# jnez71/lqRRT

Hardware: AMD Instinct MI355X
Metric: tree-node extensions/sec, 6-DoF boat, 10k-node tree (higher is better)
Workload: dtype f64; 1 GPU; demo_boat_advanced_10k; wave_cap=256, wave_cap_cli=1024, semantics=exact-sequential, parallelism=single GPU

## Files before the change

### lqrrt_amd/csrc/steer.hpp

```cpp
#pragma once

template <class S, class = void> struct is_packed : std::false_type {};
template <class S> struct is_packed<S, std::enable_if_t<S::PACKED>> : std::true_type {};

__device__ __forceinline__ bool uniform_true(bool b) { return __builtin_amdgcn_readfirstlane((int)b) != 0; }

struct SteerFuse {
    const Part* part; int n_chunks;
    NodeView nv; const double* Sd; long long s_stride;
    unsigned char* changed; unsigned char* stale; int* par_out;
    double* M; int W;
    const double* xtrig;
    int* lf0; int* round_ctl;
    double* sh_hdr; double* sh_tail; int* sh_cursor; int sh_hd, sh_tb;
};

template <class S, class = void> struct wants_two : std::false_type {};
template <class S> struct wants_two<S, std::enable_if_t<S::TWO_WAVEFRONTS>> : std::true_type {};
template <class S> constexpr int steer_wavefronts_max() { return has_dare_gain<S>::value ? 4 : is_packed<S>::value ? 3 : wants_two<S>::value ? 2 : 1; }
struct DuoLds {
    double pk[2 * MAXN + 4 + MAXM];
    double rud;
    int go, stop, cnt, steps, grew, truncated;
    int fin;
    double pk2[2][2 * MAXN + 4 + MAXM];
    double tr[2][2];
    double e2b[2];
    double tt[2];
};

template <class S>
__device__ __forceinline__ void rollout_record(const double* xn, const double* trn, const double* u, int cnt,
                                               double* hx, double* hu, double* htr) {
#pragma unroll
    for (int d = 0; d < S::N; ++d) hx[cnt * S::N + d] = xn[d];
#pragma unroll
    for (int j = 0; j < S::M; ++j) hu[cnt * S::M + j] = u[j];
#pragma unroll
    for (int j = 0; j < 2 * S::NW; ++j) htr[2 * S::NW * cnt + j] = trn[j];
}
template <class S>
__device__ __forceinline__ bool rollout_check(const double* Pl, const Geo& g, const GeoL& gl, const Res& r, const double* xn,
                                              const double* trn, const double* e, const double* u, int lane, int& cnt, int& steps,
                                              double* last, const double* tolr, double* hx, double* hu, double* htr, DuoLds& duo,
                                              bool* rec_later = nullptr, const bool* feas_known = nullptr) {
    bool stop = false;
    const bool feas_ok = feas_known ? *feas_known : uniform_true(S::feasible(Pl, g, gl, xn, u, trn, lane));
    if (!feas_ok) {
        cnt = (int)(r.FPR * (double)cnt);
        duo.truncated = 1;
        stop = true;
    } else {
        ++steps;
        if (r.adaptive) {
            bool all_grew = true;
#pragma unroll
            for (int d = 0; d < S::N; ++d) all_grew = all_grew && (fabs(e[d]) >= last[d]);
            if (uniform_true(all_grew)) { cnt = 0; duo.grew = 1; stop = true; }
#pragma unroll
            for (int d = 0; d < S::N; ++d) last[d] = fabs(e[d]);
        }
        if (!stop) {
            bool conv = true;
#pragma unroll
            for (int d = 0; d < S::N; ++d) conv = conv && (fabs(e[d]) <= tolr[d]);
            if (steps > r.H || uniform_true(conv)) {
                stop = true;
            } else {
                if (rec_later) *rec_later = true;
                else { rollout_record<S>(xn, trn, u, cnt, hx, hu, htr); ++cnt; }
            }
        }
    }
    if (stop) { duo.cnt = cnt; duo.steps = steps; duo.stop = 1; }
    return stop;
}

template <class S, int DENSE, int NWF, bool KERNARG_TOUCH>
__device__ __forceinline__ void steer_body(const Params& P, const Geo& g, const Res& r, const TreeView& tv, double* __restrict__ rec,
                                           const RecLayout& L, const double* __restrict__ xs,
                                           const int* __restrict__ list, const int lo,
                                           const int* __restrict__ par, const int* __restrict__ list_count,
                                           const SteerFuse& f, const RoundArgs& ra, const int rd_on, const int rd_round, const int rd_W, const int rd_base, const int rd_seq, const long long rd_max_commit, const long long rd_room, const int bid) {
    const bool ron = rd_on != 0;
    if (list_count && bid + lo >= list_count[0]) return;
#ifndef LQRRT_NO_KERNARG_TOUCH
    if constexpr (KERNARG_TOUCH) {
        const volatile int* ka = (const volatile int*)__builtin_amdgcn_kernarg_segment_ptr();
        constexpr int KA_LINES = (int)((sizeof(Params) + sizeof(Geo) + sizeof(Res) + sizeof(TreeView) + sizeof(RecLayout) +
                                        sizeof(SteerFuse) + sizeof(RoundArgs) + 40) / 64);
        if ((int)(threadIdx.x & 63) < KA_LINES) (void)ka[(threadIdx.x & 63) * 16];
    }
#endif
    STEER_TS(0);
    BLK_T(blk_t0);
    constexpr bool COOP = has_dare_gain<S>::value && NWF == 4;
    constexpr int GNT = COOP ? 256 : 64;
    constexpr bool DUO = NWF >= 2 && !COOP;
    static_assert(NWF <= 2 || is_packed<S>::value || COOP, "the chain rollout needs the duo_* / *_effort pieces of the system");
    static_assert(!has_dare_gain<S>::value || NWF == 1 || NWF == 4, "Riccati systems: one wavefront, or four that share the gain");
    constexpr bool PLAIN2 = NWF == 2 && !is_packed<S>::value;
    extern __shared__ double hist[];
    double* hx = hist;
    double* hu = hist + (size_t)r.H * S::N;
    const int lane = threadIdx.x & 63;
    __shared__ double Pl[MAXP];
    __shared__ double tol_l[MAXN], glo_l[MAXN], ghi_l[MAXN];
    __shared__ double node_l[MAXN + 4 + MAXM * MAXN];
    __shared__ GainLds<S> gl_lds;
    __shared__ DuoLds duo;
    double* htr = hist + (size_t)r.H * (S::N + S::M) + geo_lds_doubles(g);
    constexpr int PKN = S::N + 2 * S::NW;
    constexpr bool CH = NWF == 3 && is_packed<S>::value;
    if constexpr (CH) {
        if (threadIdx.x >= 128) {
            if (ron && !ra.gblk && ra.ctl[RC_CONV + (rd_round & 1)]) return;
            for (int i = lane; i < MAXP; i += 64) Pl[i] = P.p[i];
            if (lane < MAXN) { tol_l[lane] = r.tol[lane]; glo_l[lane] = r.goal_lo[lane]; ghi_l[lane] = r.goal_hi[lane]; }
            const GeoL gl = stage_geo(g, hist + (size_t)r.H * (S::N + S::M), lane, 64);
            __syncthreads();
            if (!duo.go) return;
            double tolr[S::N], last[S::N];
#pragma unroll
            for (int d = 0; d < S::N; ++d) { tolr[d] = tol_l[d]; last[d] = INFINITY; }
            int cnt = 0, steps = 0;
            bool stopped = false;
            for (int p = 1;; ++p) {
                __syncthreads();
                if (stopped) return;
                STEP_TS(cs0);
                double xn[S::N], trn[2], e[S::N], u[S::M];
                const double* pk = duo.pk2[p & 1];
#pragma unroll
                for (int d = 0; d < S::N; ++d) { xn[d] = pk[d]; e[d] = pk[S::N + d]; }
#pragma unroll
                for (int j = 0; j < S::M; ++j) u[j] = pk[2 * S::N + j];
                trn[0] = duo.tr[p & 1][0]; trn[1] = duo.tr[p & 1][1];
                bool rec_now = false;
                stopped = rollout_check<S>(Pl, g, gl, r, xn, trn, e, u, lane, cnt, steps, last, tolr, hx, hu, htr, duo, &rec_now);
                if (rec_now) { rollout_record<S>(xn, trn, u, cnt, hx, hu, htr); ++cnt; }
                STEP_TS(cs1);
                STEP_ACC(5, cs0, cs1);
            }
        }
        if (threadIdx.x >= 64) {
            if (ron && !ra.gblk && ra.ctl[RC_CONV + (rd_round & 1)]) return;
            __syncthreads();
            if (!duo.go) return;
            const double tt0 = duo.tt[0], tt1 = duo.tt[1];
            for (int p = 0;; ++p) {
                STEP_TS(ds0);
                const double hn = duo.pk2[p & 1][2] + duo.pk2[p & 1][5] * r.dt;
                double tn[2];
                lq_sincos(hn, &tn[1], &tn[0]);
                duo.tr[(p + 1) & 1][0] = tn[0]; duo.tr[(p + 1) & 1][1] = tn[1];
                duo.e2b[(p + 1) & 1] = lq_atan2(tt1 * tn[0] - tt0 * tn[1], tt0 * tn[0] + tt1 * tn[1]);
                STEP_TS(ds1);
                STEP_ACC(7, ds0, ds1);
                __syncthreads();
                if (duo.stop) return;
            }
        }
    }
    if constexpr (PLAIN2) {
        if (threadIdx.x >= 64) {
            if (ron && !ra.gblk && ra.ctl[RC_CONV + (rd_round & 1)]) return;
            for (int i = lane; i < MAXP; i += 64) Pl[i] = P.p[i];
            if (lane < MAXN) { tol_l[lane] = r.tol[lane]; glo_l[lane] = r.goal_lo[lane]; ghi_l[lane] = r.goal_hi[lane]; }
            const GeoL gl = stage_geo(g, hist + (size_t)r.H * (S::N + S::M), lane, 64);
            __syncthreads();
            if (!duo.go) return;
            double tolr[S::N], last[S::N];
#pragma unroll
            for (int d = 0; d < S::N; ++d) { tolr[d] = tol_l[d]; last[d] = INFINITY; }
            int cnt = 0, steps = 0;
            for (int k = 0;; ++k) {
                __syncthreads();
                if (duo.stop) return;
                double xn[S::N], trn[2 * S::NW + 1], e[S::N], u[S::M];
                const double* pk = duo.pk2[k & 1];
#pragma unroll
                for (int d = 0; d < S::N; ++d) { xn[d] = pk[d]; e[d] = pk[PKN + d]; }
#pragma unroll
                for (int j = 0; j < 2 * S::NW; ++j) trn[j] = pk[S::N + j];
#pragma unroll
                for (int j = 0; j < S::M; ++j) u[j] = pk[PKN + S::N + j];
                rollout_check<S>(Pl, g, gl, r, xn, trn, e, u, lane, cnt, steps, last, tolr, hx, hu, htr, duo);
            }
        }
    }
    if constexpr (NWF == 2 && !PLAIN2) {
        if (threadIdx.x >= 64) {
            if (ron && !ra.gblk && ra.ctl[RC_CONV + (rd_round & 1)]) return;
            for (int i = lane; i < MAXP; i += 64) Pl[i] = P.p[i];
            if (lane < MAXN) { tol_l[lane] = r.tol[lane]; glo_l[lane] = r.goal_lo[lane]; ghi_l[lane] = r.goal_hi[lane]; }
            const GeoL gl = stage_geo(g, hist + (size_t)r.H * (S::N + S::M), lane, 64);
            __syncthreads();
            if (!duo.go) return;
            double tolr[S::N], last[S::N];
#pragma unroll
            for (int d = 0; d < S::N; ++d) { tolr[d] = tol_l[d]; last[d] = INFINITY; }
            int cnt = 0, steps = 0;
            for (int k = 0;; ++k) {
                double xn[S::N], trn[2], e[S::N], u[S::M];
                STEP_TS(hs0);
#pragma unroll
                for (int d = 0; d < S::N; ++d) { xn[d] = duo.pk[d]; e[d] = duo.pk[S::N + 2 + d]; }
                trn[0] = duo.pk[S::N]; trn[1] = duo.pk[S::N + 1];
#pragma unroll
                for (int j = 0; j < S::M; ++j) u[j] = duo.pk[2 * S::N + 2 + j];
                if (!duo.fin) duo.rud = S::duo_chain(Pl, xn, trn);
                STEP_TS(hs1);
                __syncthreads();
                STEP_TS(hs2);
                if (k >= 1) {
                    bool stop = false;
                    const bool feas_ok = uniform_true(S::feasible(Pl, g, gl, xn, u, trn, lane));
                    if (!feas_ok) {
                        cnt = (int)(r.FPR * (double)cnt);
                        duo.truncated = 1;
                        stop = true;
                    } else {
                        ++steps;
                        if (r.adaptive) {
                            bool all_grew = true;
#pragma unroll
                            for (int d = 0; d < S::N; ++d) all_grew = all_grew && (fabs(e[d]) >= last[d]);
                            if (uniform_true(all_grew)) { cnt = 0; duo.grew = 1; stop = true; }
#pragma unroll
                            for (int d = 0; d < S::N; ++d) last[d] = fabs(e[d]);
                        }
                        if (!stop) {
                            bool conv = true;
#pragma unroll
                            for (int d = 0; d < S::N; ++d) conv = conv && (fabs(e[d]) <= tolr[d]);
                            if (steps > r.H || uniform_true(conv)) {
                                stop = true;
                            } else {
#pragma unroll
                                for (int d = 0; d < S::N; ++d) hx[cnt * S::N + d] = xn[d];
#pragma unroll
                                for (int j = 0; j < S::M; ++j) hu[cnt * S::M + j] = u[j];
                                htr[2 * cnt] = trn[0]; htr[2 * cnt + 1] = trn[1];
                                ++cnt;
                            }
                        }
                    }
                    if (stop) { duo.cnt = cnt; duo.steps = steps; duo.stop = 1; }
                }
                STEP_TS(hs3);
                __syncthreads();
                STEP_TS(hs4);
                STEP_ACC(0, hs0, hs1); STEP_ACC(1, hs1, hs2); STEP_ACC(2, hs2, hs3); STEP_ACC(4, hs3, hs4); STEP_ACC(3, hs0, hs0 + 1);
                if (duo.stop) return;
            }
        }
    }
    const int t = list ? list[bid + (list_count ? lo : 0)] : lo + bid;
    double* my = rec + (size_t)t * L.R;

    double x[S::N], K[S::M * S::N], trig[2 * S::NW + 1], xt[S::N], ttrig[2 * S::NW + 1];
#pragma unroll
    for (int d = 0; d < S::N; ++d) xt[d] = xs[(size_t)t * S::N + d];
    if (f.xtrig) {
#pragma unroll
        for (int j = 0; j < 2 * S::NW; ++j) ttrig[j] = f.xtrig[(size_t)t * (2 * S::NW) + j];
    } else {
        trig_of<S>(xt, ttrig);
    }
    bool parent_loaded = false;
    constexpr int HD = S::N + 2 * S::NW + S::M * S::N;
    int psel = 0;
    int head_out = 0;
    auto load_parent = [&](int p) {
        if (p >= 0) {
#pragma unroll
            for (int d = 0; d < S::N; ++d) x[d] = tv.state[(size_t)d * tv.cap + p];
#pragma unroll
            for (int j = 0; j < 2 * S::NW; ++j) trig[j] = tv.trig[(size_t)j * tv.cap + p];
#pragma unroll
            for (int j = 0; j < S::M * S::N; ++j) K[j] = tv.K[(size_t)p * S::M * S::N + j];
        } else {
            const double* hp = (ron && ra.gblk) ? gathered_header(ra, ~p) + L.off_xend
                             : (ron && psel)    ? ra.head2 + (size_t)(~p) * HD
                                                : rec + (size_t)(~p) * L.R + L.off_xend;
#pragma unroll
            for (int d = 0; d < S::N; ++d) x[d] = hp[d];
#pragma unroll
            for (int j = 0; j < 2 * S::NW; ++j) trig[j] = hp[S::N + j];
#pragma unroll
            for (int j = 0; j < S::M * S::N; ++j) K[j] = hp[S::N + 2 * S::NW + j];
        }
// ... 116 lines not shown
            stale_t = ra.stale[cur][t];
        }
        auto flags_of = [&](int idx) -> int {
            int v = 0;
#pragma unroll
            for (int i = 0; i < 4; ++i) { const int w = __shfl((int)chg[i], idx & 63); if ((idx >> 6) == i) v = w; }
            return v;
        };
        auto changed_of = [&](int idx) -> bool { return (flags_of(idx) & 1) != 0; };
        auto sel_of = [&](int idx) -> int { return (flags_of(idx) >> 1) & 1; };
        const int sel_t = sel_of(t);
        if (conv_flag) {
            const int C = ra.ctl[RC_C];
            const int len = ra.lf[cur][2 * t];
            if (t < C && len > 0) {
                const int id = rd_base + ra.rank[t];
                const double* hd = sel_t ? ra.head2 + (size_t)t * HD : my + L.off_xend;
                if (lane < S::N) tv.state[(size_t)lane * tv.cap + id] = hd[lane];
                if (lane < 2 * S::NW) tv.trig[(size_t)lane * tv.cap + id] = hd[S::N + lane];
                if constexpr (S::NW > 0) {
                    if (ra.fx.on && lane >= 32 && lane < 32 + S::NW) {
                        const int kk = lane - 32;
                        tv.werr[(size_t)kk * tv.cap + id] = wrap_err(ra.fx.t[2 * kk], ra.fx.t[2 * kk + 1], hd[S::N + 2 * kk], hd[S::N + 2 * kk + 1]);
                    }
                }
                for (int q = lane; q < S::M * S::N; q += 64) tv.K[(size_t)id * S::M * S::N + q] = hd[S::N + 2 * S::NW + q];
                if (lane == 0) {
                    const int p = ra.par[cur][t];
                    tv.pID[id] = p >= 0 ? p : rd_base + ra.rank[~p];
                    tv.elen[id] = len;
                }
                double* xe = tv.xedge + (size_t)id * tv.H * S::N;
                double* ue = tv.uedge + (size_t)id * tv.H * S::M;
                for (int q = lane; q < len * S::N; q += 64) xe[q] = my[L.off_xseq + q];
                for (int q = lane; q < len * S::M; q += 64) ue[q] = my[L.off_useq + q];
            }
            return;
        }
        int want = par_t;
        bool need = false, defer = false, mark_stale = false;
        int hz = rd_W - 1;
#pragma unroll
        for (int i = 0; i < 4; ++i)
            if (hz == rd_W - 1 && lf_len[i] > 0 && (lf_flg[i] & 1)) hz = lane + 64 * i;
#pragma unroll
        for (int off = 32; off > 0; off >>= 1) hz = min(hz, __shfl_xor(hz, off));
        if (t <= hz) {
            double wc = INFINITY;
            int sm = -1;
#pragma unroll
            for (int i = 0; i < 4; ++i)
                if (lane + 64 * i < t && colv[i] < wc) { wc = colv[i]; sm = lane + 64 * i; }
            lexmin_wave(wc, sm);
            want = (sm >= 0 && wc < csnap_t) ? ~sm : psnap_t;
            need = (want != par_t) || (stale_t != 0);
            if (want < 0 && changed_of(~want)) need = true;
            if (need) { psel = want < 0 ? sel_of(~want) : 0; load_parent(want); parent_loaded = true; }
            if (need && want < 0) {
                const int sn = ~want;
                const double* Mc = ra.M[cur];
                const double* hs = g0 ? gathered_header(ra, sn) : nullptr;
                double cs[4];
#pragma unroll
                for (int i = 0; i < 4; ++i)
                    cs[i] = (lane + 64 * i < sn) ? (g0 ? hcost(gathered_header(ra, lane + 64 * i), sn) : Mc[(size_t)(lane + 64 * i) * rd_W + sn]) : INFINITY;
                const double csnap_s = g0 ? hs[L.off_cost] : rec[(size_t)sn * L.R + L.off_cost];
                const int psnap_s = g0 ? (int)hs[L.off_parent] : (int)rec[(size_t)sn * L.R + L.off_parent];
                const int par_s = g0 ? psnap_s : ra.par[cur][sn];
                const int stale_s = g0 ? (((int)hs[L.off_len] > 0 && (int)hs[L.off_xseq] < 0) ? 1 : 0) : ra.stale[cur][sn];
                double ws = INFINITY;
                int ss = -1;
#pragma unroll
                for (int i = 0; i < 4; ++i)
                    if (lane + 64 * i < sn && cs[i] < ws) { ws = cs[i]; ss = lane + 64 * i; }
                lexmin_wave(ws, ss);
                const int want_s = (ss >= 0 && ws < csnap_s) ? ~ss : psnap_s;
                bool need_s = (want_s != par_s) || (stale_s != 0);
                if (want_s < 0 && changed_of(~want_s)) need_s = true;
                defer = need_s;
                if (defer) {
                    double wc2 = INFINITY;
                    int sm2 = -1;
#pragma unroll
                    for (int i = 0; i < 4; ++i) {
                        const int c = lane + 64 * i;
                        const double v = (c < t && c != sn) ? (g0 ? colv[i] : Mc[(size_t)c * rd_W + t]) : INFINITY;
                        if (v < wc2) { wc2 = v; sm2 = c; }
                    }
                    lexmin_wave(wc2, sm2);
                    const int want2 = (sm2 >= 0 && wc2 < csnap_t) ? ~sm2 : psnap_t;
                    if (want2 != par_t || stale_t != 0) {
                        want = want2; defer = false;
                        psel = want2 < 0 ? sel_of(~want2) : 0;
                        parent_loaded = false;
                    }
                }
            }
        } else if (want < 0 && changed_of(~want)) {
            mark_stale = true;
        }
        const bool redo = need && !defer;
        head_out = g0 ? 0 : (redo ? sel_t ^ 1 : sel_t);
        if (lane == 0) {
            ra.par[nxt][t] = redo ? want : par_t;
            ra.stale[nxt][t] = redo ? 0 : ((need && defer) || mark_stale ? 1 : stale_t);
            ra.changed[nxt][t] = (unsigned char)((redo ? 1 : 0) | (head_out << 1));
        }
        if (redo) round_share += RC_ONE_LIST;
        else if (need) round_share += RC_ONE_DEFER;
        {
            unsigned long long* word_r = (unsigned long long*)(ra.ctl + RC_PACK) + cur;
            if (threadIdx.x == 0) round_before = __hip_atomic_fetch_add(word_r, round_share, __ATOMIC_RELAXED, __HIP_MEMORY_SCOPE_AGENT);
        }
        if (!redo) {
            if (g0) {
                const double* ht = gathered_header(ra, t);
                for (int u = t + 1 + lane; u < rd_W; u += 64) ra.M[nxt][(size_t)t * rd_W + u] = hcost(ht, u);
                if (lane < 2) ra.lf[nxt][2 * t + lane] = (int)ht[lane == 0 ? L.off_len : L.off_flags];
            } else {
                for (int u = t + 1 + lane; u < rd_W; u += 64) ra.M[nxt][(size_t)t * rd_W + u] = ra.M[cur][(size_t)t * rd_W + u];
                if (lane < 2) ra.lf[nxt][2 * t + lane] = ra.lf[cur][2 * t + lane];
            }
            pref = 0x7fffffff;
        } else {
            pref = want;
        }
    } else {
        pref = par[t];
    }
    BLK_T(blk_tp);
    const bool round_skip = ron && pref == 0x7fffffff;
    if constexpr (DUO) {
        if (round_skip) { duo.go = 0; __syncthreads(); }
    }
    if (!round_skip) {
    if (!parent_loaded) load_parent(pref);

    STEER_TS(1);
    BLK_T(blk_tq);
    int cnt = 0, steps = 0;
    bool grew = false, truncated = false;
    if constexpr (CH) {
        duo.go = 1; duo.stop = 0; duo.cnt = 0; duo.steps = 0; duo.grew = 0; duo.truncated = 0;
#pragma unroll
        for (int d = 0; d < S::N; ++d) duo.pk2[0][d] = x[d];
        duo.tr[0][0] = trig[0]; duo.tr[0][1] = trig[1];
        duo.tt[0] = ttrig[0]; duo.tt[1] = ttrig[1];
        __syncthreads();
        BLK_T(blk_t1);
        STEER_T_PROLOGUE(f.n_chunks > 0 ? 0 : (ron ? 1 : 2), blk_t0, blk_tp, blk_tq, blk_t1);
        double Pc[S::NP];
#pragma unroll
        for (int i = 0; i < S::NP; ++i) Pc[i] = Pl[i];
        for (int p = 0;; ++p) {
            STEP_TS(ms0);
            double e[S::N], u[S::M], xn[S::N];
            if (p >= 1) {
                trig[0] = duo.tr[p & 1][0]; trig[1] = duo.tr[p & 1][1];
                const double e2 = duo.e2b[p & 1];
                S::gain(Pc, x, trig, x, K);
                S::quad_effort(xt, x, K, e2, e, u);
            } else {
                S::trio_effort(xt, ttrig, x, trig, K, e, u);
            }
            const double rud = S::duo_chain(Pc, x, trig);
            S::duo_finish(Pc, x, trig, u, rud, r.dt, xn);
            double* pk = duo.pk2[(p + 1) & 1];
#pragma unroll
            for (int d = 0; d < S::N; ++d) { pk[d] = xn[d]; pk[S::N + d] = e[d]; x[d] = xn[d]; }
#pragma unroll
            for (int j = 0; j < S::M; ++j) pk[2 * S::N + j] = u[j];
            STEP_TS(ms1);
            __syncthreads();
            STEP_TS(ms4);
            STEP_ACC(0, ms0, ms1); STEP_ACC(4, ms1, ms4); STEP_ACC(3, ms0, ms0 + 1);
            if (duo.stop) break;
        }
        cnt = duo.cnt; steps = duo.steps; grew = duo.grew != 0;
        truncated = true;
        STEER_T_LOOP(steps, blk_t0, blk_t1);
    } else if constexpr (PLAIN2) {
        duo.go = 1; duo.stop = 0; duo.cnt = 0; duo.steps = 0; duo.grew = 0; duo.truncated = 0;
        __syncthreads();
        double tolr[S::N];
#pragma unroll
        for (int d = 0; d < S::N; ++d) tolr[d] = tol_l[d];
        bool live = true;
        for (int k = 0;; ++k) {
            if (live) {
                double e[S::N], u[S::M], uc[S::M], xn[S::N], trn[2 * S::NW + 1];
                erf_cached<S>(xt, ttrig, x, trig, e);
#pragma unroll
                for (int i = 0; i < S::M; ++i) {
                    double a = K[i * S::N] * e[0];
#pragma unroll
                    for (int j = 1; j < S::N; ++j) a += K[i * S::N + j] * e[j];
                    u[i] = a; uc[i] = a;
                }
                S::step(Pl, x, trig, uc, r.dt, xn);
                trig_of<S>(xn, trn);
                double* pk = duo.pk2[k & 1];
#pragma unroll
                for (int d = 0; d < S::N; ++d) { pk[d] = xn[d]; pk[PKN + d] = e[d]; x[d] = xn[d]; }
#pragma unroll
                for (int j = 0; j < 2 * S::NW; ++j) { pk[S::N + j] = trn[j]; trig[j] = trn[j]; }
#pragma unroll
                for (int j = 0; j < S::M; ++j) pk[PKN + S::N + j] = u[j];
                system_gain<S>(Pl, x, trig, u, r.dt, gl_lds, lane, K);
                bool conv = true;
#pragma unroll
                for (int d = 0; d < S::N; ++d) conv = conv && (fabs(e[d]) <= tolr[d]);
                if (k + 1 > r.H || uniform_true(conv)) live = false;
            }
            __syncthreads();
            if (duo.stop) break;
        }
        cnt = duo.cnt; steps = duo.steps; grew = duo.grew != 0;
        truncated = true;
    } else if constexpr (NWF == 2) {
        duo.go = 1; duo.stop = 0; duo.cnt = 0; duo.steps = 0; duo.grew = 0; duo.truncated = 0; duo.fin = 0;
#pragma unroll
        for (int d = 0; d < S::N; ++d) duo.pk[d] = x[d];
        duo.pk[S::N] = trig[0]; duo.pk[S::N + 1] = trig[1];
        __syncthreads();
        double tolr[S::N];
#pragma unroll
        for (int d = 0; d < S::N; ++d) tolr[d] = tol_l[d];
        bool live = true;
        for (int k = 0;; ++k) {
            double e[S::N], u[S::M], xn[S::N], trn[2];
            if (live) {
                S::duo_effort(xt, ttrig, x, trig, K, r.dt, e, u, trn);
                S::gain(Pl, x, trn, u, K);
            }
            __syncthreads();
            if (live) {
                const double rud = duo.rud;
                S::duo_finish(Pl, x, trig, u, rud, r.dt, xn);
#pragma unroll
                for (int d = 0; d < S::N; ++d) { duo.pk[d] = xn[d]; duo.pk[S::N + 2 + d] = e[d]; x[d] = xn[d]; }
                duo.pk[S::N] = trn[0]; duo.pk[S::N + 1] = trn[1];
                trig[0] = trn[0]; trig[1] = trn[1];
#pragma unroll
                for (int j = 0; j < S::M; ++j) duo.pk[2 * S::N + 2 + j] = u[j];
                bool conv = true;
#pragma unroll
                for (int d = 0; d < S::N; ++d) conv = conv && (fabs(e[d]) <= tolr[d]);
                if (k + 1 > r.H || uniform_true(conv)) { duo.fin = 1; live = false; }
            }
            __syncthreads();
            if (duo.stop) break;
        }
        cnt = duo.cnt; steps = duo.steps; grew = duo.grew != 0;
        truncated = true;
    } else {
    for (int i = lane; i < MAXP; i += 64) Pl[i] = P.p[i];
    if (lane < MAXN) { tol_l[lane] = r.tol[lane]; glo_l[lane] = r.goal_lo[lane]; ghi_l[lane] = r.goal_hi[lane]; }
    const GeoL gl = stage_geo(g, hist + (size_t)r.H * (S::N + S::M), lane, 64);
    __syncthreads();
    STEER_TS(2);
    double tolr[S::N];
#pragma unroll
    for (int d = 0; d < S::N; ++d) tolr[d] = tol_l[d];
    double last[S::N];
#pragma unroll
    for (int d = 0; d < S::N; ++d) last[d] = INFINITY;
    while (true) {
        double e[S::N], u[S::M], uc[S::M], xn[S::N], trn[2 * S::NW + 1];
        STEP_TS(ts0);
        if constexpr (is_packed<S>::value) {
            S::step_packed(Pl, xt, ttrig, x, trig, K, r.dt, lane, e, u, xn, trn);
        } else {
            erf_cached<S>(xt, ttrig, x, trig, e);
#pragma unroll
            for (int i = 0; i < S::M; ++i) {
                double a = K[i * S::N] * e[0];
#pragma unroll
                for (int j = 1; j < S::N; ++j) a += K[i * S::N + j] * e[j];
                u[i] = a; uc[i] = a;
            }
            S::step(Pl, x, trig, uc, r.dt, xn);
            trig_of<S>(xn, trn);
        }
        STEP_TS(ts1);
        const bool feas_ok = uniform_true(S::feasible(Pl, g, gl, xn, u, trn, lane));
        STEP_TS(ts2);
        STEP_ACC(0, ts0, ts1); STEP_ACC(1, ts1, ts2);
        if (!feas_ok) {
            cnt = (int)(r.FPR * (double)cnt);
            truncated = true;
            break;
        }
        ++steps;
        if (r.adaptive) {
            bool all_grew = true;
#pragma unroll
            for (int d = 0; d < S::N; ++d) all_grew = all_grew && (fabs(e[d]) >= last[d]);
            if (uniform_true(all_grew)) { cnt = 0; grew = true; break; }
#pragma unroll
            for (int d = 0; d < S::N; ++d) last[d] = fabs(e[d]);
        }
        bool conv = true;
#pragma unroll
        for (int d = 0; d < S::N; ++d) conv = conv && (fabs(e[d]) <= tolr[d]);
        if (steps > r.H || uniform_true(conv)) break;
        {
#pragma unroll
            for (int d = 0; d < S::N; ++d) hx[cnt * S::N + d] = xn[d];
#pragma unroll
            for (int j = 0; j < S::M; ++j) hu[cnt * S::M + j] = u[j];
        }
        ++cnt;
#pragma unroll
        for (int d = 0; d < S::N; ++d) x[d] = xn[d];
#pragma unroll
        for (int j = 0; j < 2 * S::NW; ++j) trig[j] = trn[j];
        system_gain<S, GNT>(Pl, x, trig, u, r.dt, gl_lds, COOP ? (int)threadIdx.x : lane, K);
        STEP_TS(ts3);
        STEP_ACC(2, ts2, ts3); STEP_ACC(3, ts0, ts0 + 1);
    }
    }
    STEER_TS(3);
    __syncthreads();

// ... 95 lines not shown
```

### lqrrt_amd/csrc/systems.hpp

```cpp
#pragma once
#include <hip/hip_runtime.h>
#include <math.h>
#include "../../include/lqrrt_pmath.h"

namespace lq {

constexpr int MAXN = 12;
constexpr int MAXM = 6;
constexpr int MAXP = 96;

struct Params { double p[MAXP]; };

struct Geo {
    const double* vps;
    const double* obs;
    const double* oc;
    const int* cell_start;
    const int* cell_items;
    double glo[3], ghi[3], gcell;
    int gdim[3];
    int V, O, stride, pad;
    const signed char* og;
    double og_ox, og_oy, og_cpm, og_thr;
    int og_rows, og_cols;
    const unsigned char* ogc;
    int ogc_rows, ogc_cols, og_lds;
    double og_reach;
    double og_bb[4];
    double hbb[4];
};
constexpr int OG_COARSE_SHIFT = 3;

struct GeoL {
    const double* vps;
    const double* oc;
    int V, O;
    double bb[4];
};

__device__ __forceinline__ size_t geo_lds_doubles(const Geo& g) {
    if (g.og) return g.og_lds ? (size_t)2 * g.V : 0;
    return g.oc ? (size_t)2 * g.V + (size_t)4 * g.O : 0;
}

__device__ __forceinline__ GeoL stage_geo(const Geo& g, double* lds, int tid, int nthreads) {
    GeoL L;
    L.V = g.V; L.O = g.O;
    L.vps = lds; L.oc = lds + 2 * g.V;
#pragma unroll
    for (int k = 0; k < 4; ++k) L.bb[k] = g.hbb[k];
    if (g.og) {
        if (g.og_lds) { for (int i = tid; i < 2 * g.V; i += nthreads) lds[i] = g.vps[i]; }
        else L.vps = g.vps;
        return L;
    }
    if (g.oc) {
        for (int i = tid; i < 2 * g.V; i += nthreads) lds[i] = g.vps[i];
        for (int i = tid; i < 4 * g.O; i += nthreads) lds[2 * g.V + i] = g.oc[i];
    }
    return L;
}

__device__ __forceinline__ double clipd(double v, double lo, double hi) {
    double t = v < lo ? lo : v;
    return t > hi ? hi : t;
}

template <int Q>
__device__ __forceinline__ double quad_bcast(double v) {
    int lo = __double2loint(v), hi = __double2hiint(v);
    lo = __builtin_amdgcn_mov_dpp(lo, Q * 0x55, 0xf, 0xf, true);
    hi = __builtin_amdgcn_mov_dpp(hi, Q * 0x55, 0xf, 0xf, true);
    return __hiloint2double(hi, lo);
}

__device__ __forceinline__ double wrap_err(double cg, double sg, double c, double s) {
    return lq_atan2(sg * c - cg * s, cg * c + sg * s);
}
__device__ __forceinline__ double wrap_err_c(double cg, double sg, double c, double s) {
    return lq_atan2_c(sg * c - cg * s, cg * c + sg * s);
}

template <int n>
__device__ __forceinline__ double numpy_row_sum(const double* a) {
    if constexpr (n < 8) {
        double r = a[0];
#pragma unroll
        for (int i = 1; i < n; ++i) r += a[i];
        return r;
    } else {
        double r0 = a[0], r1 = a[1], r2 = a[2], r3 = a[3], r4 = a[4], r5 = a[5], r6 = a[6], r7 = a[7];
        int i = 8;
        for (; i < n - (n % 8); i += 8) {
            r0 += a[i + 0]; r1 += a[i + 1]; r2 += a[i + 2]; r3 += a[i + 3];
            r4 += a[i + 4]; r5 += a[i + 5]; r6 += a[i + 6]; r7 += a[i + 7];
        }
        double res = ((r0 + r1) + (r2 + r3)) + ((r4 + r5) + (r6 + r7));
        for (; i < n; ++i) res += a[i];
        return res;
    }
}

__device__ __forceinline__ bool grid_hits(const Geo& g, const GeoL& gl, double px, double py, double c, double s, int lane) {
    {
        const double x0 = g.og_cpm * ((px - g.og_reach) - g.og_ox), x1 = g.og_cpm * ((px + g.og_reach) - g.og_ox);
        const double y0 = g.og_cpm * ((py - g.og_reach) - g.og_oy), y1 = g.og_cpm * ((py + g.og_reach) - g.og_oy);
        if (x0 >= 2.0 && y0 >= 2.0 && x1 < (double)(g.og_cols - 2) && y1 < (double)(g.og_rows - 2)) {
            const int cx0 = ((int)x0 - 1) >> OG_COARSE_SHIFT, cx1 = ((int)x1 + 1) >> OG_COARSE_SHIFT;
            const int cy0 = ((int)y0 - 1) >> OG_COARSE_SHIFT, cy1 = ((int)y1 + 1) >> OG_COARSE_SHIFT;
            const int nx = cx1 - cx0 + 1, cells = nx * (cy1 - cy0 + 1);
            bool occ = false;
            for (int q = lane; q < cells; q += 64) {
                const int r = q / nx, cc = q - r * nx;
                occ |= g.ogc[(size_t)(cy0 + r) * g.ogc_cols + (cx0 + cc)] != 0;
            }
            if (__any(occ) == 0) return false;
            const double ax0 = c * g.og_bb[0], ax1 = c * g.og_bb[1], bx0 = s * g.og_bb[0], bx1 = s * g.og_bb[1];
            const double ay0 = s * g.og_bb[2], ay1 = s * g.og_bb[3], by0 = c * g.og_bb[2], by1 = c * g.og_bb[3];
            const double wx_lo = fmin(ax0, ax1) - fmax(ay0, ay1), wx_hi = fmax(ax0, ax1) - fmin(ay0, ay1);
            const double wy_lo = fmin(bx0, bx1) + fmin(by0, by1), wy_hi = fmax(bx0, bx1) + fmax(by0, by1);
            const double m = 1e-9 * (1.0 + g.og_reach);
            const int fx0 = (int)(g.og_cpm * ((px + wx_lo - m) - g.og_ox)) - 1, fx1 = (int)(g.og_cpm * ((px + wx_hi + m) - g.og_ox)) + 1;
            const int fy0 = (int)(g.og_cpm * ((py + wy_lo - m) - g.og_oy)) - 1, fy1 = (int)(g.og_cpm * ((py + wy_hi + m) - g.og_oy)) + 1;
            const int fnx = fx1 - fx0 + 1, fcells = fnx * (fy1 - fy0 + 1);
            if (fcells <= 1024 && fx0 >= 0 && fy0 >= 0 && fx1 < g.og_cols && fy1 < g.og_rows) {
                bool focc = false;
                for (int q = lane; q < fcells; q += 64) {
                    const int r = q / fnx, cc = q - r * fnx;
                    focc |= !((double)g.og[(size_t)(fy0 + r) * g.og_cols + (fx0 + cc)] < g.og_thr);
                }
                if (__any(focc) == 0) return false;
            }
        }
    }
    bool hit = false;
    const double ms = -s;
    for (int v0 = lane; v0 < g.V; v0 += 8 * 64) {
        long long cell[8];
        bool oob[8], live[8];
#pragma unroll
        for (int k = 0; k < 8; ++k) {
            const int v = v0 + 64 * k;
            live[k] = v < g.V;
            const int vv = live[k] ? v : lane;
            const double bx = gl.vps[vv], by = gl.vps[g.V + vv];
            const double vx = px + (c * bx + ms * by);
            const double vy = py + (s * bx + c * by);
            const double fx = g.og_cpm * (vx - g.og_ox), fy = g.og_cpm * (vy - g.og_oy);
            const bool wild = !(fabs(fx) < 0x1p63) || !(fabs(fy) < 0x1p63);
            long long ix = (long long)fx;
            long long iy = (long long)fy;
            if (ix < 0) ix += g.og_cols;
            if (iy < 0) iy += g.og_rows;
            oob[k] = wild || ix < 0 || ix >= g.og_cols || iy < 0 || iy >= g.og_rows;
            cell[k] = oob[k] ? 0 : iy * g.og_cols + ix;
        }
        signed char val[8];
#pragma unroll
        for (int k = 0; k < 8; ++k) val[k] = g.og[cell[k]];
#pragma unroll
        for (int k = 0; k < 8; ++k) hit |= live[k] && (oob[k] || !((double)val[k] < g.og_thr));
    }
    return __any(hit) != 0;
}

__device__ __forceinline__ bool hull_hits(const GeoL& g, double px, double py, double c, double s,
                                          bool extra2p, int lane) {
    ABL_IF_NOFEAS(return false;)
    bool hit = false;
    const double ms = -s;
    for (int o0 = 0; o0 < g.O; o0 += 64) {
        const int o = o0 + lane;
        bool near = false;
        if (o < g.O) {
            const double ox = g.oc[4 * o], oy = g.oc[4 * o + 1], rp = g.oc[4 * o + 3];
            const double dx = ox - px, dy = oy - py;
            const double cbx = c * dx + s * dy, cby = c * dy + ms * dx;
            near = (cbx >= g.bb[0] - rp) && (cbx <= g.bb[1] + rp) && (cby >= g.bb[2] - rp) && (cby <= g.bb[3] + rp);
            if (extra2p) {
                const double ex = (px + px) - ox, ey = (py + py) - oy;
                hit |= (ex * ex + ey * ey) <= g.oc[4 * o + 2];
            }
        }
        unsigned long long m = __ballot(near);
        while (m) {
            const int j = __builtin_ctzll(m);
            m &= m - 1;
            const double ox = g.oc[4 * (o0 + j)], oy = g.oc[4 * (o0 + j) + 1], thr = g.oc[4 * (o0 + j) + 2];
            for (int v = lane; v < g.V; v += 64) {
                const double bx = g.vps[v], by = g.vps[g.V + v];
                const double vx = px + (c * bx + ms * by);
                const double vy = py + (s * bx + c * by);
                const double dx = vx - ox, dy = vy - oy;
                hit |= (dx * dx + dy * dy) <= thr;
            }
        }
    }
    return __any(hit) != 0;
}


struct BoatCommon {
    static constexpr int N = 6, M = 3, NW = 1;
    __host__ __device__ __forceinline__ static constexpr int wd(int) { return 2; }

    __device__ __forceinline__ static void gain_pd(const double* kp, const double* kd, const double* trig, double* K) {
        const double c = trig[0], s = trig[1];
        K[0] = kp[0] * c;    K[1] = kp[0] * s;  K[2] = kp[0] * 0.0;  K[3] = kd[0]; K[4] = 0.0;   K[5] = 0.0;
        K[6] = kp[1] * (-s); K[7] = kp[1] * c;  K[8] = kp[1] * 0.0;  K[9] = 0.0;   K[10] = kd[1]; K[11] = 0.0;
        K[12] = kp[2] * 0.0; K[13] = kp[2] * 0.0; K[14] = kp[2] * 1.0; K[15] = 0.0; K[16] = 0.0;  K[17] = kd[2];
    }

    __device__ __forceinline__ static bool torque_direct(double vmin2, const double* x) {
        return x[3] >= 0.0 && x[3] * x[3] + x[4] * x[4] > vmin2;
    }
    __device__ __forceinline__ static double rudder_ref(double gainv, const double* x, double c, double s) {
        const double vw0 = c * x[3] + (-s) * x[4];
        const double vw1 = s * x[3] + c * x[4];
        const double ang = lq_atan2(vw1, vw0);
        double cg, sg;
        lq_sincos(ang, &sg, &cg);
        return gainv * wrap_err(cg, sg, c, s);
    }
    __device__ __forceinline__ static double rudder_term(double gainv, double vmin2, const double* x, double c, double s) {
        ABL_IF_NORUDDER(return 0.0;)
        if (torque_direct(vmin2, x)) return gainv * lq_atan2(x[4], x[3]);
        return rudder_ref(gainv, x, c, s);
    }

    __device__ __forceinline__ static void packed_heading(double gainv, const double* ttrig, const double* x, const double* trig,
                                          double dt, int lane, double yb, double xb, bool direct, double& e2, double& rud, double* trn) {
        const bool odd = (lane & 1) != 0;
        const double c = trig[0], s = trig[1];
        const double ya = ttrig[1] * c - ttrig[0] * s, xa = ttrig[0] * c + ttrig[1] * s;
        ABL_IF_NORUDDER(e2 = lq_atan2(ya, xa); rud = 0.0; lq_sincos(x[2] + x[5] * dt, &trn[1], &trn[0]); return;)
        ABL_IF_NOTRIG(e2 = ya; rud = yb * 1e-3; trn[1] = s; trn[0] = c; return;)
        const double hn = x[2] + x[5] * dt;
        if (__builtin_amdgcn_readfirstlane((int)direct)) {
            const double a = lq_atan2(odd ? x[4] : ya, odd ? x[3] : xa);
            e2 = quad_bcast<0>(a);
            rud = gainv * quad_bcast<1>(a);
            lq_sincos(hn, &trn[1], &trn[0]);
            return;
        }
        const double a = lq_atan2(odd ? yb : ya, odd ? xb : xa);
        e2 = quad_bcast<0>(a);
        const double ang = quad_bcast<1>(a);
        double sn, cs;
        lq_sincos(odd ? hn : ang, &sn, &cs);
        const double sg = quad_bcast<0>(sn), cg = quad_bcast<0>(cs);
        trn[1] = quad_bcast<1>(sn);
        trn[0] = quad_bcast<1>(cs);
        rud = gainv * wrap_err(cg, sg, c, s);
    }

    __device__ __forceinline__ static void packed_erf_effort(double gainv, const double* xt, const double* ttrig, const double* x,
                                             const double* trig, const double* K, double dt, int lane, double yb, double xb,
                                             bool direct, double* e, double* u, double& rud, double* trn) {
        double e2;
        packed_heading(gainv, ttrig, x, trig, dt, lane, yb, xb, direct, e2, rud, trn);
#pragma unroll
        for (int d = 0; d < 6; ++d) e[d] = xt[d] - x[d];
        e[2] = e2;
#pragma unroll
        for (int i = 0; i < 3; ++i) {
            double a = K[i * 6] * e[0];
#pragma unroll
            for (int j = 1; j < 6; ++j) a += K[i * 6 + j] * e[j];
            u[i] = a;
        }
    }

    __device__ __forceinline__ static void duo_effort(const double* xt, const double* ttrig, const double* x, const double* trig,
                                      const double* K, double dt, double* e, double* u, double* trn) {
        const double c = trig[0], s = trig[1];
#pragma unroll
        for (int d = 0; d < 6; ++d) e[d] = xt[d] - x[d];
        e[2] = lq_atan2(ttrig[1] * c - ttrig[0] * s, ttrig[0] * c + ttrig[1] * s);
#pragma unroll
        for (int i = 0; i < 3; ++i) {
            double a = K[i * 6] * e[0];
#pragma unroll
            for (int j = 1; j < 6; ++j) a += K[i * 6 + j] * e[j];
            u[i] = a;
        }
        lq_sincos(x[2] + x[5] * dt, &trn[1], &trn[0]);
    }
    __device__ __forceinline__ static void trio_effort(const double* xt, const double* ttrig, const double* x, const double* trig,
                                       const double* K, double* e, double* u) {
        const double c = trig[0], s = trig[1];
#pragma unroll
        for (int d = 0; d < 6; ++d) e[d] = xt[d] - x[d];
        e[2] = lq_atan2(ttrig[1] * c - ttrig[0] * s, ttrig[0] * c + ttrig[1] * s);
#pragma unroll
        for (int i = 0; i < 3; ++i) {
            double a = K[i * 6] * e[0];
#pragma unroll
            for (int j = 1; j < 6; ++j) a += K[i * 6 + j] * e[j];
            u[i] = a;
        }
    }
    __device__ __forceinline__ static void quad_effort(const double* xt, const double* x, const double* K, double e2, double* e, double* u) {
#pragma unroll
        for (int d = 0; d < 6; ++d) e[d] = xt[d] - x[d];
        e[2] = e2;
#pragma unroll
        for (int i = 0; i < 3; ++i) {
            double a = K[i * 6] * e[0];
#pragma unroll
            for (int j = 1; j < 6; ++j) a += K[i * 6 + j] * e[j];
            u[i] = a;
        }
    }
    __device__ __forceinline__ static double duo_rudder(double gainv, double yb, double xb, double c, double s) {
        const double ang = lq_atan2(yb, xb);
        double cg, sg;
        lq_sincos(ang, &sg, &cg);
        return gainv * wrap_err(cg, sg, c, s);
    }

    __device__ __forceinline__ static void euler(const double* invM, const double* Dpos, const double* Dneg,
                                 const double* x, double c, double s, const double* u, double dt, double* xn) {
        double xdot[6];
        xdot[0] = c * x[3] + (-s) * x[4];
        xdot[1] = s * x[3] + c * x[4];
        xdot[2] = x[5];
#pragma unroll
        for (int i = 0; i < 3; ++i) {
            const double v = x[3 + i];
            const double D = (v >= 0.0) ? Dpos[i] : Dneg[i];
            xdot[3 + i] = invM[i] * (u[i] - D * v);
        }
#pragma unroll
        for (int i = 0; i < 6; ++i) xn[i] = x[i] + xdot[i] * dt;
    }

    __device__ __forceinline__ static void carlike(const double* x, double vpos0, double vneg0, double* xn) {
        if (x[3] > 0.0)      xn[5] = clipd(fabs(xn[3] / vpos0), 0.0, 1.0) * xn[5];
        else if (x[3] < 0.0) xn[5] = clipd(fabs(xn[3] / vneg0), 0.0, 1.0) * xn[5];
        if (xn[3] < 0.0) xn[3] = 0.0;
    }
};

struct BoatAdvanced : BoatCommon {
    __device__ __forceinline__ static void gain(const double* P, const double*, const double* trig, const double*, double* K) {
        gain_pd(P + 40, P + 43, trig, K);
    }
    static constexpr bool PACKED = true;
    static constexpr int NP = 53;
    __device__ __forceinline__ static void step(const double* P, const double* x, const double* trig, double* u, double dt, double* xn) {
        u[2] = u[2] + rudder_term(P[37], P[52], x, trig[0], trig[1]);
        thrust_and_integrate(P, x, trig, u, dt, xn);
    }
    __device__ __forceinline__ static void step_packed(const double* P, const double* xt, const double* ttrig, const double* x,
                                       const double* trig, const double* K, double dt, int lane,
                                       double* e, double* u, double* xn, double* trn) {
        const double c = trig[0], s = trig[1];
        const double vw0 = c * x[3] + (-s) * x[4];
        const double vw1 = s * x[3] + c * x[4];
        double rud;
        packed_erf_effort(P[37], xt, ttrig, x, trig, K, dt, lane, vw1, vw0, torque_direct(P[52], x), e, u, rud, trn);
        double uc[3] = {u[0], u[1], u[2] + rud};
        thrust_and_integrate(P, x, trig, uc, dt, xn);
    }
    __device__ __forceinline__ static double duo_chain(const double* P, const double* x, const double* trig) {
        return rudder_term(P[37], P[52], x, trig[0], trig[1]);
    }
    __device__ __forceinline__ static void duo_finish(const double* P, const double* x, const double* trig, const double* u, double rud, double dt, double* xn) {
        double uc[3] = {u[0], u[1], u[2] + rud};
        thrust_and_integrate(P, x, trig, uc, dt, xn);
    }
    __device__ __forceinline__ static void thrust_and_integrate(const double* P, const double* x, const double* trig, double* u, double dt, double* xn) {
        const double c = trig[0], s = trig[1];
        double t[4];
#pragma unroll
        for (int j = 0; j < 4; ++j) {
            double a = P[21 + 3 * j] * u[0];
            a += P[21 + 3 * j + 1] * u[1];
            a += P[21 + 3 * j + 2] * u[2];
            t[j] = clipd(a, -P[33 + j], P[33 + j]);
        }
        double us[3];
#pragma unroll
        for (int i = 0; i < 3; ++i) {
            double a = P[9 + 4 * i] * t[0];
            a += P[9 + 4 * i + 1] * t[1];
            a += P[9 + 4 * i + 2] * t[2];
            a += P[9 + 4 * i + 3] * t[3];
            us[i] = a;
        }
        euler(P + 0, P + 3, P + 6, x, c, s, us, dt, xn);
        carlike(x, P[38], P[39], xn);
    }
    __device__ __forceinline__ static bool feasible(const double* P, const Geo& g, const GeoL& gl, const double* x, const double*, const double* trig, int lane) {
#pragma unroll
        for (int i = 0; i < 3; ++i)
            if (x[3 + i] > P[46 + i] || x[3 + i] < P[49 + i]) return false;
        if (g.og) return !grid_hits(g, gl, x[0], x[1], trig[0], trig[1], lane);
        return !hull_hits(gl, x[0], x[1], trig[0], trig[1], false, lane);
    }
};

struct BoatIntermediate : BoatCommon {
    __device__ __forceinline__ static void gain(const double* P, const double*, const double* trig, const double*, double* K) {
        gain_pd(P + 15, P + 18, trig, K);
    }
    static constexpr bool PACKED = true;
    static constexpr int NP = 22;
    __device__ __forceinline__ static void step(const double* P, const double* x, const double* trig, double* u, double dt, double* xn) {
        u[2] = u[2] + rudder_term(P[12], P[21], x, trig[0], trig[1]);
        saturate_and_integrate(P, x, trig, u, dt, xn);
    }
    __device__ __forceinline__ static void step_packed(const double* P, const double* xt, const double* ttrig, const double* x,
                                       const double* trig, const double* K, double dt, int lane,
                                       double* e, double* u, double* xn, double* trn) {
        const double c = trig[0], s = trig[1];
        const double vw0 = c * x[3] + (-s) * x[4];
        const double vw1 = s * x[3] + c * x[4];
        double rud;
        packed_erf_effort(P[12], xt, ttrig, x, trig, K, dt, lane, vw1, vw0, torque_direct(P[21], x), e, u, rud, trn);
        double uc[3] = {u[0], u[1], u[2] + rud};
        saturate_and_integrate(P, x, trig, uc, dt, xn);
    }
    __device__ __forceinline__ static double duo_chain(const double* P, const double* x, const double* trig) {
        return rudder_term(P[12], P[21], x, trig[0], trig[1]);
    }
    __device__ __forceinline__ static void duo_finish(const double* P, const double* x, const double* trig, const double* u, double rud, double dt, double* xn) {
        double uc[3] = {u[0], u[1], u[2] + rud};
        saturate_and_integrate(P, x, trig, uc, dt, xn);
    }
    __device__ __forceinline__ static void saturate_and_integrate(const double* P, const double* x, const double* trig, double* u, double dt, double* xn) {
#pragma unroll
        for (int i = 0; i < 3; ++i)
            if (fabs(u[i]) > P[9 + i]) u[i] = P[9 + i] * (u[i] > 0.0 ? 1.0 : -1.0);
        euler(P + 0, P + 3, P + 6, x, trig[0], trig[1], u, dt, xn);
        carlike(x, P[13], P[14], xn);
    }
    __device__ __forceinline__ static bool feasible(const double*, const Geo& g, const GeoL& gl, const double* x, const double*, const double* trig, int lane) {
        if (g.og) return !grid_hits(g, gl, x[0], x[1], trig[0], trig[1], lane);
        return !hull_hits(gl, x[0], x[1], trig[0], trig[1], false, lane);
    }
};

struct BoatNovice : BoatCommon {
    static constexpr bool TWO_WAVEFRONTS = true;
    __device__ __forceinline__ static void gain(const double* P, const double*, const double* trig, const double*, double* K) {
        gain_pd(P + 12, P + 15, trig, K);
    }
    __device__ __forceinline__ static void step(const double* P, const double* x, const double* trig, double* u, double dt, double* xn) {
#pragma unroll
        for (int i = 0; i < 3; ++i)
            if (fabs(u[i]) > P[9 + i]) u[i] = P[9 + i] * (u[i] > 0.0 ? 1.0 : -1.0);
        euler(P + 0, P + 3, P + 6, x, trig[0], trig[1], u, dt, xn);
    }
    __device__ __forceinline__ static bool feasible(const double*, const Geo&, const GeoL& gl, const double* x, const double*, const double*, int lane) {
        bool hit = false;
        for (int o = lane; o < gl.O; o += 64) {
            const double dx = x[0] - gl.oc[4 * o], dy = x[1] - gl.oc[4 * o + 1];
            hit |= (dx * dx + dy * dy) <= gl.oc[4 * o + 2];
        }
        return __any(hit) == 0;
    }
};

struct RosBoat : BoatCommon {
    __device__ __forceinline__ static void gain(const double* P, const double*, const double* trig, const double*, double* K) {
        gain_pd(P + 43, P + 46, trig, K);
    }
    static constexpr bool PACKED = true;
    static constexpr int NP = 50;
    __device__ __forceinline__ static void step(const double* P, const double* x, const double* trig, double* u, double dt, double* xn) {
        const double c = trig[0], s = trig[1];
        const int rmode = (int)P[38];
        if (rmode == 1) {
            const double ang = lq_atan2(P[40] - x[1], P[39] - x[0]);
            double cg, sg;
            lq_sincos(ang, &sg, &cg);
            u[2] = P[37] * wrap_err(cg, sg, c, s);
        } else if (rmode == 2) {
            u[2] = rudder_term(P[37], P[49], x, c, s);
        }
        thrust_and_integrate(P, x, trig, u, dt, xn);
    }
    __device__ __forceinline__ static void step_packed(const double* P, const double* xt, const double* ttrig, const double* x,
                                       const double* trig, const double* K, double dt, int lane,
                                       double* e, double* u, double* xn, double* trn) {
        const int rmode = (int)P[38];
        if (rmode == 0) {
#pragma unroll
            for (int d = 0; d < 6; ++d) e[d] = xt[d] - x[d];
            e[2] = wrap_err(ttrig[0], ttrig[1], trig[0], trig[1]);
            double uc[3];
#pragma unroll
            for (int i = 0; i < 3; ++i) {
                double a = K[i * 6] * e[0];
#pragma unroll
                for (int j = 1; j < 6; ++j) a += K[i * 6 + j] * e[j];
                u[i] = a; uc[i] = a;
            }
            thrust_and_integrate(P, x, trig, uc, dt, xn);
            lq_sincos(xn[2], &trn[1], &trn[0]);
            return;
        }
        const double c = trig[0], s = trig[1];
        double yb, xb;
        if (rmode == 1) { yb = P[40] - x[1]; xb = P[39] - x[0]; }
        else { xb = c * x[3] + (-s) * x[4]; yb = s * x[3] + c * x[4]; }
        double rud;
        packed_erf_effort(P[37], xt, ttrig, x, trig, K, dt, lane, yb, xb, rmode == 2 && torque_direct(P[49], x), e, u, rud, trn);
        double uc[3] = {u[0], u[1], rud};
        thrust_and_integrate(P, x, trig, uc, dt, xn);
    }
    __device__ __forceinline__ static double duo_chain(const double* P, const double* x, const double* trig) {
        const int rmode = (int)P[38];
        if (rmode == 0) return 0.0;
        const double c = trig[0], s = trig[1];
        double yb, xb;
        if (rmode == 2) return rudder_term(P[37], P[49], x, c, s);
        yb = P[40] - x[1]; xb = P[39] - x[0];
        return duo_rudder(P[37], yb, xb, c, s);
    }
    __device__ __forceinline__ static void duo_finish(const double* P, const double* x, const double* trig, const double* u, double rud, double dt, double* xn) {
        double uc[3] = {u[0], u[1], (int)P[38] == 0 ? u[2] : rud};
// ... 191 lines not shown
```

Baseline: 682,700 extension attempts/s.

## Split boat thrust integration across quad lanes and restructure hull collision loop

Adds a chain_step path for BoatAdvanced that spreads the thrust-allocation and velocity-integration rows across the four lanes of a quad and gathers the results with quad broadcasts. The per-lane parameter rows are hoisted out of the step loop. The rudder torque branch is made wave-uniform via readfirstlane, and carlike clipping becomes branchless. Separately, hull_hits is restructured to loop over vertices in the outer loop, read obstacle data from registers via readlane, and access vertices through LDS address-space pointers. The checker wavefront also caches parameters in registers, and the main loop skips step work once p exceeds the horizon. The readfirstlane uniformization assumes all lanes agree on torque_direct, which may not hold exactly.

```diff
diff --git a/lqrrt_amd/csrc/steer.hpp b/lqrrt_amd/csrc/steer.hpp
--- a/lqrrt_amd/csrc/steer.hpp
+++ b/lqrrt_amd/csrc/steer.hpp
@@ -17,6 +17,15 @@
 
 template <class S, class = void> struct wants_two : std::false_type {};
 template <class S> struct wants_two<S, std::enable_if_t<S::TWO_WAVEFRONTS>> : std::true_type {};
+struct NoChainRows {};
+template <class S, class = void> struct chain_step : std::false_type {
+    using Rows = NoChainRows;
+    __device__ __forceinline__ static Rows rows(const double*, int) { return {}; }
+};
+template <class S> struct chain_step<S, std::enable_if_t<S::CHAIN_STEP>> : std::true_type {
+    using Rows = typename S::ChainRows;
+    __device__ __forceinline__ static Rows rows(const double* P, int lane) { return S::chain_rows(P, lane); }
+};
 template <class S> constexpr int steer_wavefronts_max() { return has_dare_gain<S>::value ? 4 : is_packed<S>::value ? 3 : wants_two<S>::value ? 2 : 1; }
 struct DuoLds {
     double pk[2 * MAXN + 4 + MAXM];
@@ -123,6 +132,9 @@
             double tolr[S::N], last[S::N];
 #pragma unroll
             for (int d = 0; d < S::N; ++d) { tolr[d] = tol_l[d]; last[d] = INFINITY; }
+            double Pc[S::NP];
+#pragma unroll
+            for (int i = 0; i < S::NP; ++i) Pc[i] = Pl[i];
             int cnt = 0, steps = 0;
             bool stopped = false;
             for (int p = 1;; ++p) {
@@ -137,7 +149,7 @@
                 for (int j = 0; j < S::M; ++j) u[j] = pk[2 * S::N + j];
                 trn[0] = duo.tr[p & 1][0]; trn[1] = duo.tr[p & 1][1];
                 bool rec_now = false;
-                stopped = rollout_check<S>(Pl, g, gl, r, xn, trn, e, u, lane, cnt, steps, last, tolr, hx, hu, htr, duo, &rec_now);
+                stopped = rollout_check<S>(Pc, g, gl, r, xn, trn, e, u, lane, cnt, steps, last, tolr, hx, hu, htr, duo, &rec_now);
                 if (rec_now) { rollout_record<S>(xn, trn, u, cnt, hx, hu, htr); ++cnt; }
                 STEP_TS(cs1);
                 STEP_ACC(5, cs0, cs1);
@@ -560,24 +572,32 @@
         double Pc[S::NP];
 #pragma unroll
         for (int i = 0; i < S::NP; ++i) Pc[i] = Pl[i];
+        [[maybe_unused]] const typename chain_step<S>::Rows rows = chain_step<S>::rows(Pl, lane);
         for (int p = 0;; ++p) {
             STEP_TS(ms0);
-            double e[S::N], u[S::M], xn[S::N];
-            if (p >= 1) {
-                trig[0] = duo.tr[p & 1][0]; trig[1] = duo.tr[p & 1][1];
-                const double e2 = duo.e2b[p & 1];
-                S::gain(Pc, x, trig, x, K);
-                S::quad_effort(xt, x, K, e2, e, u);
-            } else {
-                S::trio_effort(xt, ttrig, x, trig, K, e, u);
-            }
-            const double rud = S::duo_chain(Pc, x, trig);
-            S::duo_finish(Pc, x, trig, u, rud, r.dt, xn);
-            double* pk = duo.pk2[(p + 1) & 1];
-#pragma unroll
-            for (int d = 0; d < S::N; ++d) { pk[d] = xn[d]; pk[S::N + d] = e[d]; x[d] = xn[d]; }
-#pragma unroll
-            for (int j = 0; j < S::M; ++j) pk[2 * S::N + j] = u[j];
+            if (p <= r.H) {
+                double e[S::N], u[S::M], xn[S::N];
+                if (p >= 1) {
+                    trig[0] = duo.tr[p & 1][0]; trig[1] = duo.tr[p & 1][1];
+                    const double e2 = duo.e2b[p & 1];
+                    S::gain(Pc, x, trig, x, K);
+                    S::quad_effort(xt, x, K, e2, e, u);
+                } else {
+                    S::trio_effort(xt, ttrig, x, trig, K, e, u);
+                }
+                if constexpr (chain_step<S>::value) {
+                    const double rud = S::chain_torque(Pc, x, trig);
+                    S::chain_finish(Pc, rows, lane, x, trig, u, rud, r.dt, xn);
+                } else {
+                    const double rud = S::duo_chain(Pc, x, trig);
+                    S::duo_finish(Pc, x, trig, u, rud, r.dt, xn);
+                }
+                double* pk = duo.pk2[(p + 1) & 1];
+#pragma unroll
+                for (int d = 0; d < S::N; ++d) { pk[d] = xn[d]; pk[S::N + d] = e[d]; x[d] = xn[d]; }
+#pragma unroll
+                for (int j = 0; j < S::M; ++j) pk[2 * S::N + j] = u[j];
+            }
             STEP_TS(ms1);
             __syncthreads();
             STEP_TS(ms4);
diff --git a/lqrrt_amd/csrc/systems.hpp b/lqrrt_amd/csrc/systems.hpp
--- a/lqrrt_amd/csrc/systems.hpp
+++ b/lqrrt_amd/csrc/systems.hpp
@@ -164,35 +164,44 @@
     return __any(hit) != 0;
 }
 
+__device__ __forceinline__ double lane_read(double v, int j) {
+    const int lo = __builtin_amdgcn_readlane(__double2loint(v), j), hi = __builtin_amdgcn_readlane(__double2hiint(v), j);
+    return __hiloint2double(hi, lo);
+}
+
 __device__ __forceinline__ bool hull_hits(const GeoL& g, double px, double py, double c, double s,
                                           bool extra2p, int lane) {
     ABL_IF_NOFEAS(return false;)
     bool hit = false;
     const double ms = -s;
+    const __attribute__((address_space(3))) double* vps = (const __attribute__((address_space(3))) double*)g.vps;
     for (int o0 = 0; o0 < g.O; o0 += 64) {
         const int o = o0 + lane;
         bool near = false;
+        double ox = 0.0, oy = 0.0, thr = 0.0;
         if (o < g.O) {
-            const double ox = g.oc[4 * o], oy = g.oc[4 * o + 1], rp = g.oc[4 * o + 3];
+            ox = g.oc[4 * o]; oy = g.oc[4 * o + 1]; thr = g.oc[4 * o + 2];
+            const double rp = g.oc[4 * o + 3];
             const double dx = ox - px, dy = oy - py;
             const double cbx = c * dx + s * dy, cby = c * dy + ms * dx;
             near = (cbx >= g.bb[0] - rp) && (cbx <= g.bb[1] + rp) && (cby >= g.bb[2] - rp) && (cby <= g.bb[3] + rp);
             if (extra2p) {
                 const double ex = (px + px) - ox, ey = (py + py) - oy;
-                hit |= (ex * ex + ey * ey) <= g.oc[4 * o + 2];
-            }
-        }
-        unsigned long long m = __ballot(near);
-        while (m) {
-            const int j = __builtin_ctzll(m);
-            m &= m - 1;
-            const double ox = g.oc[4 * (o0 + j)], oy = g.oc[4 * (o0 + j) + 1], thr = g.oc[4 * (o0 + j) + 2];
-            for (int v = lane; v < g.V; v += 64) {
-                const double bx = g.vps[v], by = g.vps[g.V + v];
-                const double vx = px + (c * bx + ms * by);
-                const double vy = py + (s * bx + c * by);
-                const double dx = vx - ox, dy = vy - oy;
-                hit |= (dx * dx + dy * dy) <= thr;
+                hit |= (ex * ex + ey * ey) <= thr;
+            }
+        }
+        const unsigned long long m = __ballot(near);
+        if (m == 0) continue;
+        for (int v0 = 0; v0 < g.V; v0 += 64) {
+            const bool live = v0 + lane < g.V;
+            const int v = live ? v0 + lane : 0;
+            const double bx = vps[v], by = vps[g.V + v];
+            const double vx = px + (c * bx + ms * by);
+            const double vy = py + (s * bx + c * by);
+            for (unsigned long long mm = m; mm; mm &= mm - 1) {
+                const int j = __builtin_ctzll(mm);
+                const double dx = vx - lane_read(ox, j), dy = vy - lane_read(oy, j);
+                hit |= live && (dx * dx + dy * dy) <= lane_read(thr, j);
             }
         }
     }
@@ -225,6 +234,11 @@
     __device__ __forceinline__ static double rudder_term(double gainv, double vmin2, const double* x, double c, double s) {
         ABL_IF_NORUDDER(return 0.0;)
         if (torque_direct(vmin2, x)) return gainv * lq_atan2(x[4], x[3]);
+        return rudder_ref(gainv, x, c, s);
+    }
+    __device__ __forceinline__ static double rudder_term_uniform(double gainv, double vmin2, const double* x, double c, double s) {
+        ABL_IF_NORUDDER(return 0.0;)
+        if (__builtin_amdgcn_readfirstlane((int)torque_direct(vmin2, x))) return gainv * lq_atan2(x[4], x[3]);
         return rudder_ref(gainv, x, c, s);
     }
 
@@ -340,6 +354,12 @@
         else if (x[3] < 0.0) xn[5] = clipd(fabs(xn[3] / vneg0), 0.0, 1.0) * xn[5];
         if (xn[3] < 0.0) xn[3] = 0.0;
     }
+    __device__ __forceinline__ static void carlike_straight(const double* x, double vpos0, double vneg0, double* xn) {
+        const bool pos = x[3] > 0.0, neg = x[3] < 0.0;
+        const double scaled = clipd(fabs(xn[3] / (pos ? vpos0 : vneg0)), 0.0, 1.0) * xn[5];
+        xn[5] = (pos || neg) ? scaled : xn[5];
+        if (xn[3] < 0.0) xn[3] = 0.0;
+    }
 };
 
 struct BoatAdvanced : BoatCommon {
@@ -369,6 +389,45 @@
     __device__ __forceinline__ static void duo_finish(const double* P, const double* x, const double* trig, const double* u, double rud, double dt, double* xn) {
         double uc[3] = {u[0], u[1], u[2] + rud};
         thrust_and_integrate(P, x, trig, uc, dt, xn);
+    }
+    static constexpr bool CHAIN_STEP = true;
+    __device__ __forceinline__ static double chain_torque(const double* P, const double* x, const double* trig) {
+        return rudder_term_uniform(P[37], P[52], x, trig[0], trig[1]);
+    }
+    struct ChainRows { double ib0, ib1, ib2, tlo, thi, b0, b1, b2, b3, invM, Dpos, Dneg; };
+    __device__ __forceinline__ static ChainRows chain_rows(const double* P, int lane) {
+        const int q = lane & 3, i = q < 3 ? q : 2;
+        ChainRows w;
+        w.ib0 = P[21 + 3 * q]; w.ib1 = P[21 + 3 * q + 1]; w.ib2 = P[21 + 3 * q + 2];
+        w.thi = P[33 + q]; w.tlo = -P[33 + q];
+        w.b0 = P[9 + 4 * i]; w.b1 = P[9 + 4 * i + 1]; w.b2 = P[9 + 4 * i + 2]; w.b3 = P[9 + 4 * i + 3];
+        w.invM = P[i]; w.Dpos = P[3 + i]; w.Dneg = P[6 + i];
+        return w;
+    }
+    __device__ __forceinline__ static void chain_finish(const double* P, const ChainRows& w, int lane, const double* x, const double* trig,
+                                                        const double* u, double rud, double dt, double* xn) {
+        const double c = trig[0], s = trig[1];
+        const double u2 = u[2] + rud;
+        double a = w.ib0 * u[0];
+        a += w.ib1 * u[1];
+        a += w.ib2 * u2;
+        const double tq = clipd(a, w.tlo, w.thi);
+        const double t0 = quad_bcast<0>(tq), t1 = quad_bcast<1>(tq), t2 = quad_bcast<2>(tq), t3 = quad_bcast<3>(tq);
+        double us = w.b0 * t0;
+        us += w.b1 * t1;
+        us += w.b2 * t2;
+        us += w.b3 * t3;
+        const int q = lane & 3;
+        const double x3 = x[3], x4 = x[4], x5 = x[5];
+        const double v = q == 0 ? x3 : q == 1 ? x4 : x5;
+        const double D = (v >= 0.0) ? w.Dpos : w.Dneg;
+        const double vdot = w.invM * (us - D * v);
+        const double vn = v + vdot * dt;
+        xn[0] = x[0] + (c * x[3] + (-s) * x[4]) * dt;
+        xn[1] = x[1] + (s * x[3] + c * x[4]) * dt;
+        xn[2] = x[2] + x[5] * dt;
+        xn[3] = quad_bcast<0>(vn); xn[4] = quad_bcast<1>(vn); xn[5] = quad_bcast<2>(vn);
+        carlike_straight(x, P[38], P[39], xn);
     }
     __device__ __forceinline__ static void thrust_and_integrate(const double* P, const double* x, const double* trig, double* u, double dt, double* xn) {
         const double c = trig[0], s = trig[1];
```

Measured after the change: 738,400 extension attempts/s, median of 6. +8.2%, better.
